# richox/orz

Hardware: AMD Instinct MI355X
Metric: orz -l1 encode throughput (enwik8-shaped text, 100 MB, one 16 MiB block in flight) (higher is better)
Workload: dtype u8

## Files before the change

### include/orz_hip.h

```cpp
#ifndef ORZ_HIP_H
#define ORZ_HIP_H

#include <stddef.h>
#include <stdint.h>
#include <sys/types.h>

#ifdef __cplusplus
extern "C" {
#endif

#define ORZ_OK 0
#define ORZ_EINVAL (-22)
#define ORZ_ENOMEM (-12)
#define ORZ_EIO (-5)
#define ORZ_ENODEV (-19)
#define ORZ_EBADMSG (-74)

#define ORZ_LZ_BLOCK_SIZE ((1u << 25) - 1)
#define ORZ_SBVEC_SENTINEL_LEN 480u
#define ORZ_SBVEC_PREMATCH_LEN (ORZ_LZ_BLOCK_SIZE / 2)

typedef struct {
    size_t match_depth, lazy_match_depth1, lazy_match_depth2;
} orz_lzcfg;
// ... 176 lines not shown
                    uint64_t* dst_len, orz_read_stats* stats);

typedef struct {
    uint64_t hits, resumed, fresh, uncached, evicted;
    uint64_t cursors, bytes, budget;
} orz_cache_stats;
int orz_reader_set_cache(orz_reader*, uint64_t max_bytes);
uint64_t orz_reader_cursor_state_bytes(void);
int orz_reader_cache_stats(orz_reader*, orz_cache_stats* stats);

int orz_reader_set_planes(orz_reader*, const uint32_t* elems, size_t n_tensors);
int orz_reader_set_planes_pieces(orz_reader*, const uint32_t* elems, const uint32_t* pieces, size_t n_tensors);
int orz_reader_set_bases(orz_reader*, const void* const* bases, size_t n_tensors);
int orz_element_gather_time(int device, const void* d_planes, const void* d_base, void* d_dst, size_t count, uint32_t elem, int reps,
                            double* ms);
int orz_reader_tensor_info(orz_reader*, uint64_t* n_tensors, uint64_t* counts, uint32_t* elems, size_t cap);
int orz_reader_read_elements(orz_reader*, const uint64_t* tensor, const uint64_t* first, const uint64_t* count, size_t n_ranges,
                             uint8_t* d_dst, size_t d_cap, uint64_t* dst_len, orz_read_stats* stats);

size_t orz_huffman_stride(void);
int orz_huffman_tables(int device, const uint32_t* weights, size_t nchunks, uint8_t* lens, uint16_t* codes, double* elapsed_us);

int orz_symrank_chains(int device, uint16_t* tables, const uint32_t* gsym, const uint32_t* rstart, size_t nitems,
                       uint16_t* ranks, uint32_t* flags2, double* elapsed_us);

int orz_fast_step_path(int device, unsigned form, uint32_t n, uint32_t tile, uint32_t t_lo, uint32_t t_hi, uint32_t entry,
                       const uint8_t* wbytes, const uint32_t* ev, uint8_t* ty, uint8_t* nl, uint8_t* x0, uint8_t* x1, uint8_t* x2,
                       uint32_t* centry, uint32_t* tentry, uint64_t* sbits, uint8_t* pt, uint32_t* cm, uint64_t* lds_bytes);
int orz_fast_step_counts(int device, uint32_t n, const uint8_t* wbytes, const uint64_t* sbits, int count, uint32_t s0, uint32_t s1,
                         uint32_t ext, uint32_t cpt, uint32_t live_end, uint32_t rows, uint32_t* cm, uint32_t* cp, uint32_t* cp2,
                         uint32_t* ord, uint32_t* ord2, uint32_t* acc2);
int orz_fast_step_horizon(int device, const uint32_t* cp, uint32_t rows, const uint32_t* hpre, uint32_t s0, uint32_t s1, uint32_t* hz,
                          uint32_t* hz2);

int orz_device_count(void);
const char* orz_last_error(void);
const char* orz_version(void);

#ifdef __cplusplus
}
#endif
#endif
```

### orz_amd/_native.py

```python
import ctypes
import os

_HERE = os.path.dirname(os.path.abspath(__file__))
LIB_PATH = os.environ.get("ORZ_LIB_PATH") or os.path.join(_HERE, "lib", "liborz_hip.so")


class LZCfg(ctypes.Structure):

    _fields_ = [
        ("match_depth", ctypes.c_size_t),
        ("lazy_match_depth1", ctypes.c_size_t),
        ("lazy_match_depth2", ctypes.c_size_t),
    ]


class EncodeStats(ctypes.Structure):
    _fields_ = [
        ("blocks", ctypes.c_uint64),
        ("sweeps", ctypes.c_uint64),
        ("seg_evals", ctypes.c_uint64),
        ("items", ctypes.c_uint64),
        ("chunks", ctypes.c_uint64),
        ("in_bytes", ctypes.c_uint64),
        ("out_bytes", ctypes.c_uint64),
# ... 306 lines not shown
    ),
    ("orz_stream_set_item_trace", ctypes.c_int, [ctypes.c_void_p, ctypes.c_int]),
    ("orz_stream_get_item_trace", ctypes.c_long, [ctypes.c_void_p, ctypes.POINTER(Item), ctypes.c_size_t]),
    ("orz_stream_set_item_patches", ctypes.c_int, [ctypes.c_void_p, ctypes.c_void_p, ctypes.c_size_t]),
    ("orz_stream_fast_tables", ctypes.c_long, [ctypes.c_void_p, ctypes.c_int, ctypes.c_char_p, ctypes.c_void_p, ctypes.c_size_t]),
    ("orz_stream_arm_repair_probe", ctypes.c_int, [ctypes.c_void_p, ctypes.c_int, ctypes.c_void_p, ctypes.c_void_p, ctypes.c_size_t]),
    ("orz_stream_repair_probe", ctypes.c_long, [ctypes.c_void_p, ctypes.c_char_p, ctypes.c_void_p, ctypes.c_size_t]),
    ("orz_huffman_stride", ctypes.c_size_t, []),
    (
        "orz_huffman_tables",
        ctypes.c_int,
        [ctypes.c_int, ctypes.c_void_p, ctypes.c_size_t, ctypes.c_void_p, ctypes.c_void_p, ctypes.POINTER(ctypes.c_double)],
    ),
    (
        "orz_symrank_chains",
        ctypes.c_int,
        [ctypes.c_int, ctypes.c_void_p, ctypes.c_void_p, ctypes.c_void_p, ctypes.c_size_t, ctypes.c_void_p, ctypes.c_void_p,
         ctypes.POINTER(ctypes.c_double)],
    ),
    (
        "orz_fast_step_path",
        ctypes.c_int,
        [ctypes.c_int, ctypes.c_uint] + [ctypes.c_uint32] * 5 + [ctypes.c_void_p] * 12 + [ctypes.POINTER(ctypes.c_uint64)],
    ),
    (
        "orz_fast_step_counts",
        ctypes.c_int,
        [ctypes.c_int, ctypes.c_uint32, ctypes.c_void_p, ctypes.c_void_p, ctypes.c_int] + [ctypes.c_uint32] * 6 + [ctypes.c_void_p] * 6,
    ),
    (
        "orz_fast_step_horizon",
        ctypes.c_int,
        [ctypes.c_int, ctypes.c_void_p, ctypes.c_uint32, ctypes.c_void_p, ctypes.c_uint32, ctypes.c_uint32, ctypes.c_void_p, ctypes.c_void_p],
    ),
    ("orz_device_count", ctypes.c_int, []),
    ("orz_last_error", ctypes.c_char_p, []),
    ("orz_version", ctypes.c_char_p, []),
]

_lib = None


def load():
    global _lib
    if _lib is not None:
        return _lib
    if not os.path.exists(LIB_PATH):
        raise RuntimeError(
            "liborz_hip.so is not built (%s missing): run `python -c 'import __graft_entry__ as g; g.build()'`" % LIB_PATH
        )
    os.environ.setdefault("GPU_MAX_HW_QUEUES", "16")
    lib = ctypes.CDLL(LIB_PATH)
    for name, restype, argtypes in SYMBOLS:
        fn = getattr(lib, name)
        fn.restype = restype
        fn.argtypes = argtypes
    _lib = lib
    return lib


def last_error():
    return load().orz_last_error().decode("utf-8", "replace")
```

### orz_amd/csrc/orz_capi.hip

```cpp
#include <cstdlib>
#include <cstring>
#include <map>
#include <memory>
#include <mutex>
#include <new>
#include <string>
#include <atomic>
#include <thread>
#include <vector>

#include "../../include/orz_hip.h"
#include "backend_hip.h"
#include "orz_decode_device.h"
#include "orz_decode_index.h"
#include "orz_decode_range.h"
#include "orz_decode_scatter.h"
#include "orz_host_decode.h"
#include "orz_planes.h"
#include "orz_read_elements.h"
#include "orz_decode_check.h"
#include "orz_stream.h"
#include "orz_fast_step.h"

namespace {
// ... 1378 lines not shown

int orz_fast_step_path(int device, unsigned form, uint32_t n, uint32_t tile, uint32_t t_lo, uint32_t t_hi, uint32_t entry,
                       const uint8_t* wbytes, const uint32_t* ev, uint8_t* ty, uint8_t* nl, uint8_t* x0, uint8_t* x1, uint8_t* x2,
                       uint32_t* centry, uint32_t* tentry, uint64_t* sbits, uint8_t* pt, uint32_t* cm, uint64_t* lds_bytes) {
    const int bad = mapped([&] { orz::fast_step_path_check(form, n, tile, t_lo, t_hi, entry, wbytes, ev, ty, nl, x0, x1, x2, centry, tentry, sbits, pt, cm); });
    if (bad) return bad;
    if (!device_ok(device)) return fail(ORZ_ENODEV, "no such HIP device");
    return mapped([&] {
        orz::HipBackend be(device);
        orz::fast_step_path(be, form, n, tile, t_lo, t_hi, entry, wbytes, ev, ty, nl, x0, x1, x2, centry, tentry, sbits, pt, cm, lds_bytes);
    });
}
int orz_fast_step_counts(int device, uint32_t n, const uint8_t* wbytes, const uint64_t* sbits, int count, uint32_t s0, uint32_t s1,
                         uint32_t ext, uint32_t cpt, uint32_t live_end, uint32_t rows, uint32_t* cm, uint32_t* cp, uint32_t* cp2,
                         uint32_t* ord, uint32_t* ord2, uint32_t* acc2) {
    const int bad = mapped([&] { orz::fast_step_counts_check(n, wbytes, sbits, s0, s1, ext, cpt, live_end, rows, cm, cp, cp2, ord, ord2, acc2); });
    if (bad) return bad;
    if (!device_ok(device)) return fail(ORZ_ENODEV, "no such HIP device");
    return mapped([&] {
        orz::HipBackend be(device);
        orz::fast_step_counts(be, n, wbytes, sbits, count, s0, s1, ext, cpt, live_end, rows, cm, cp, cp2, ord, ord2, acc2);
    });
}
int orz_fast_step_horizon(int device, const uint32_t* cp, uint32_t rows, const uint32_t* hpre, uint32_t s0, uint32_t s1, uint32_t* hz,
                          uint32_t* hz2) {
    const int bad = mapped([&] { orz::fast_step_horizon_check(cp, rows, hpre, s0, s1, hz, hz2); });
    if (bad) return bad;
    if (!device_ok(device)) return fail(ORZ_ENODEV, "no such HIP device");
    return mapped([&] {
        orz::HipBackend be(device);
        orz::fast_step_horizon(be, cp, rows, hpre, s0, s1, hz, hz2);
    });
}

int orz_symrank_chains(int device, uint16_t* tables, const uint32_t* gsym, const uint32_t* rstart, size_t nitems,
                       uint16_t* ranks, uint32_t* flags2, double* elapsed_us) {
    if (!tables || !rstart || (!gsym && nitems) || (!ranks && nitems)) return fail(ORZ_EINVAL, "bad argument");
    if (device < 0 || device >= orz_device_count()) return fail(ORZ_ENODEV, "no such HIP device");
    if (const char* why = orz::symrank_chains_invalid(tables, gsym, rstart, nitems)) return fail(ORZ_EINVAL, why);
    try {
        orz::HipBackend be(device);
        const size_t nt = (size_t)512 * orz::kSrWords;
        struct Bufs {
            orz::HipBackend& be;
            uint16_t *st = nullptr, *backup = nullptr, *rk = nullptr;
            uint32_t *gs = nullptr, *rs = nullptr, *fl = nullptr;
            ~Bufs() { be.free(st); be.free(backup); be.free(rk); be.free(gs); be.free(rs); be.free(fl); }
        } b{be};
        b.st = be.alloc<uint16_t>(nt, false);
        b.backup = be.alloc<uint16_t>(nt, false);
        b.rk = be.alloc<uint16_t>(nitems, false);
        b.gs = be.alloc<uint32_t>(nitems, false);
        b.rs = be.alloc<uint32_t>(513, false);
        b.fl = be.alloc<uint32_t>(3);
        be.h2d(b.st, tables, nt * 2);
        be.h2d(b.gs, gsym, nitems * 4);
        be.h2d(b.rs, rstart, 513 * 4);
        struct Events {
            hipEvent_t a = nullptr, b = nullptr;
            ~Events() { if (a) (void)hipEventDestroy(a); if (b) (void)hipEventDestroy(b); }
        } ev;
        ORZ_HIP_CHECK(hipEventCreate(&ev.a));
        ORZ_HIP_CHECK(hipEventCreate(&ev.b));
        ORZ_HIP_CHECK(hipEventRecord(ev.a, be.stream()));
        be.symrank(b.st, b.gs, b.rk, b.rs, (uint32_t)nitems, b.fl, b.backup, nullptr);
        ORZ_HIP_CHECK(hipEventRecord(ev.b, be.stream()));
// ... 241 lines not shown
```

### orz_amd/csrc/orz_fast.h

```cpp
#pragma once
#include "orz_kernels.h"
#include "orz_parse.h"

namespace orz {

#if !defined(__HIPCC__)
inline unsigned long long g_far_stats[4] = {0, 0, 0, 0};
#endif

constexpr uint32_t kSub = 4096;
constexpr uint32_t kSeg64 = 64;
constexpr uint32_t kNSub = kNewMax / kSub + 2;
constexpr uint32_t kEntries = 240;

constexpr uint32_t kFastK = 32;
constexpr uint32_t kHistSub = (kPre + 1) / kSub;
constexpr uint32_t kRingMargin = 4;
constexpr uint32_t kFastTile = 262144;
constexpr uint32_t kFastRounds = 4;
constexpr uint32_t kSettledTile = 393216;
constexpr uint32_t kSettledTileDeep = 262144;
constexpr uint32_t kSettledRounds = 3;

struct FastArgs {
// ... 286 lines not shown
};
struct ColScanTop {
    uint32_t* gsum;
    uint32_t rows;
    const uint32_t* out;
    const FastCtl* ctl = nullptr;
    ORZ_HD void operator()(size_t c) const {
        if (c >= 256 || passes_done(ctl)) return;
        uint32_t v = out[c];
        for (uint32_t g = 0; g * 64 < rows; g++) {
            const uint32_t t = gsum[(size_t)g * 256 + c];
            gsum[(size_t)g * 256 + c] = v;
            v += t;
        }
    }
};
struct ColScanRows {
    const uint32_t *in, *gsum;
    uint32_t rows;
    uint32_t* out;
    const FastCtl* ctl = nullptr;
    ORZ_HD void operator()(size_t tid) const {
        if (passes_done(ctl)) return;
        const uint32_t c = (uint32_t)(tid & 255), g = (uint32_t)(tid >> 8);
        if (g * 64 >= rows) return;
        uint32_t v = gsum[(size_t)g * 256 + c];
        for (uint32_t r = g * 64; r < rows && r < g * 64 + 64; r++) {
            out[(size_t)r * 256 + c] = v;
            v += in[(size_t)r * 256 + c];
        }
        if (g * 64 + 64 >= rows) out[(size_t)rows * 256 + c] = v;
    }
};
constexpr uint32_t kRecText = 12;
ORZ_D uint32_t rec_pos(uint64_t hi) { return (uint32_t)(hi >> 32); }
ORZ_D uint32_t rec_lcp(uint64_t lo_a, uint64_t hi_a, uint64_t lo_b, uint64_t hi_b) {
    const uint64_t x0 = lo_a ^ lo_b;
    if (x0) return (uint32_t)ctz64(x0) >> 3;
    const uint32_t x1 = (uint32_t)(hi_a ^ hi_b);
    return x1 ? 8 + ((uint32_t)ctz64((uint64_t)x1) >> 3) : kRecText;
}
struct FastRowsWave {
    const uint8_t* win;
    const uint32_t* epos;
    const uint64_t* stext;
    const uint8_t* rlen;
    uint32_t nent, K;
    uint8_t* rows;
    uint64_t* rdist;
    static constexpr uint32_t kOutStride = 72;
    static size_t lds_bytes(uint32_t K) { return (size_t)(64 + K) * 16 + 64 * kOutStride; }
    template <class W>
    ORZ_D void operator()(W& w) const {
        uint64_t* t0 = (uint64_t*)w.lds();
        uint64_t* t1 = t0 + (64 + K);
        uint8_t* outL = (uint8_t*)(t1 + (64 + K));
        const uint32_t lane = w.lane();
        const int64_t base = (int64_t)w.block() * 64 - K;
        for (uint32_t e = lane; e < 64 + K; e += 64) {
            const int64_t s = base + e;
            uint64_t a = 0, b = 0;
            if (s >= 0 && s < (int64_t)nent) { a = stext[2 * s]; b = stext[2 * s + 1]; }
            t0[e] = a; t1[e] = b;
        }
        w.sync();
        const uint32_t me = K + lane;
// ... 1209 lines not shown
                    const uint32_t p = kPre + i0 + t, c = hash1(a.win, p - 1), key = c * kHash + hash_entry(a.win + p);
                    if (!((rdirty[key >> 6] >> (key & 63)) & 1) && !edge[i0 + t] && cok[c]) mm &= ~(1ull << t);
                }
            }
        }
        const uint32_t mine = (uint32_t)popc64(mm) | ((uint32_t)popc64(wm) << 16);
        uint32_t v = mine;
        for (uint32_t d = 1; d < 64; d <<= 1) {
            const uint32_t t = w.shfl(v, lane >= d ? lane - d : lane);
            if (lane >= d) v += t;
        }
        const uint32_t tot = w.bcast(v, 63);
        uint32_t mo = (v - mine) & 0xffff, wo = (v - mine) >> 16;
        uint16_t* ml = mlist + (size_t)s * kSubMatches;
        uint16_t* wl = wlist + (size_t)s * kSubWords;
        while (mm) { const uint32_t t = (uint32_t)ctz64(mm); mm &= mm - 1; ml[mo++] = (uint16_t)(lane * 64 + t); }
        while (wm) { const uint32_t t = (uint32_t)ctz64(wm); wm &= wm - 1; wl[wo++] = (uint16_t)(lane * 64 + t); }
        if (lane == 0) { mcnt[s] = tot & 0xffff; wcnt[s] = tot >> 16; }
        w.sync();
        for (uint32_t c = lane; c < 256; c += 64) a.cm[(size_t)s * 256 + c] = cnt[c];
    }
};
struct FastItemTotal {
    const uint32_t* cp;
    uint32_t nsub;
    FastCtl* ctl;
    ORZ_HD void operator()(size_t c) const {
        if (c >= 256 || ctl->done) return;
        const uint32_t mine = cp[(size_t)nsub * 256 + c] - cp[c];
        atom_add32(&ctl->acc, mine);
        atom_max32(&ctl->hotacc, mine);
    }
};
struct OrdWave {
    const uint8_t* win;
    const uint64_t* sbits;
    const uint32_t* cp;
    uint32_t n;
    uint32_t* ORD;
    const FastCtl* ctl;
    static constexpr uint32_t kRow = 257;
    static size_t lds_bytes() { return (size_t)64 * kRow * 2 + 64; }
    template <class W>
    ORZ_D void operator()(W& w) const {
        if (ctl->done) return;
        uint16_t* cnt = (uint16_t*)w.lds();
        const uint32_t s = w.block(), lane = w.lane();
        uint16_t* mine = cnt + (size_t)lane * kRow;
        for (uint32_t c = 0; c < kRow; c++) mine[c] = 0;
        const uint32_t i0 = s * kSub + lane * 64;
        const uint64_t m0 = i0 < n ? sbits[i0 / 64] : 0;
        const uint8_t* b = win + kPre + i0;
        for (uint64_t m = m0; m;) {
            const uint32_t t = (uint32_t)ctz64(m);
            m &= m - 1;
            if (i0 + t < n) mine[(uint32_t)(b[(int)t - 1] & 0x7f) | ((uint32_t)is_alnum(b[(int)t - 2]) << 7)]++;
        }
        w.sync();
        for (uint32_t c = lane; c < 256; c += 64) {
            uint32_t run = 0;
            for (uint32_t r = 0; r < 64; r++) {
                const uint32_t v = cnt[(size_t)r * kRow + c];
                cnt[(size_t)r * kRow + c] = (uint16_t)run;
                run += v;
            }
        }
// ... 443 lines not shown
```

### orz_amd/csrc/orz_fast_step.h

```cpp
#pragma once
#include <stdexcept>
#include <vector>

#include "orz_fast.h"

namespace orz {

struct FastStepInvalid : std::invalid_argument {
    using std::invalid_argument::invalid_argument;
};

template <class BE>
struct StepBufs {
    BE& be;
    std::vector<void*> all;
    explicit StepBufs(BE& b) : be(b) {}
    ~StepBufs() { for (void* p : all) be.free(p); }
    template <class T> T* zeroed(size_t n) { T* p = be.template alloc<T>(n); all.push_back(p); return p; }
    template <class T> T* from(const T* src, size_t n) {
        T* p = be.template alloc<T>(n, false);
        all.push_back(p);
        be.h2d(p, src, n * sizeof(T));
        return p;
    }
// ... 98 lines not shown
    a.cp = d_cp2;
    be.launch_waves(flip_blocks(0) + 256, FlipPrefixWave{FastFlip{}, FastPrefix{a, s0, s1, ext, cpt, live_end}, 0}, FlipPrefixWave::lds_bytes());
    be.launch(256, FastItemTotal{d_cp, (uint32_t)z.nsub, ctl});
    be.launch_waves(z.nsub, OrdWave{a.win, a.sbits, d_cp, n, biased(d_ord, kPre), ctl}, OrdWave::lds_bytes());
    be.launch_waves(z.nsub, OrdWave2{a.win, a.sbits, d_cp, n, biased(d_ord2, kPre), ctl}, OrdWave2::lds_bytes());
    FastCtl h{};
    be.d2h(&h, ctl, sizeof h);
    acc2[0] = h.acc; acc2[1] = h.hotacc;
    be.d2h(cm, a.cm, ncm * 4); be.d2h(cp, d_cp, ncp * 4); be.d2h(cp2, d_cp2, ncp * 4);
    be.d2h(ord, d_ord, (size_t)n * 4); be.d2h(ord2, d_ord2, (size_t)n * 4);
}

inline void fast_step_horizon_check(const uint32_t* cp, uint32_t rows, const uint32_t* hpre, uint32_t s0, uint32_t s1, const uint32_t* hz, const uint32_t* hz2) {
    if (!cp || !hpre || !hz || !hz2) throw FastStepInvalid("null array");
    if (s0 > s1 || s1 + 2 > rows || rows > kNSub + 2) throw FastStepInvalid("subtile range");
}
template <class BE>
void fast_step_horizon(BE& be, const uint32_t* cp, uint32_t rows, const uint32_t* hpre, uint32_t s0, uint32_t s1, uint32_t* hz, uint32_t* hz2) {
    fast_step_horizon_check(cp, rows, hpre, s0, s1, hz, hz2);
    StepBufs<BE> b(be);
    FastArgs a{};
    a.cp = b.from(const_cast<uint32_t*>(cp), (size_t)rows * 256);
    a.hpre = b.from(const_cast<uint32_t*>(hpre), (size_t)(kHistSub + 1) * 256);
    const size_t nhz = ((size_t)s1 + 1) * 256 * 4;
    uint32_t* d_hz = b.from(hz, nhz);
    uint32_t* d_hz2 = b.from(hz2, nhz);
    a.hz = d_hz;
    { const FastHorizon fh{a, s0, s1}; be.launch(fh.threads(), fh); }
    a.hz = d_hz2;
    { const FastHorizon fh{a, s0, s1}; be.launch_waves((fh.threads() + 63) / 64, RetireHorizonWave{FastRetire{}, fh, 0}, 0); }
    be.d2h(hz, d_hz, nhz * 4); be.d2h(hz2, d_hz2, nhz * 4);
}

}
```

### orz_amd/csrc/orz_kernels.h

```cpp
#pragma once
#include "orz_common.h"

#if defined(__HIP_DEVICE_COMPILE__)
#define ORZ_ATOMIC_ADD(p, v) atomicAdd((p), (v))
#define ORZ_ATOMIC_MIN(p, v) atomicMin((p), (v))
#define ORZ_ATOMIC_MAX(p, v) atomicMax((p), (v))
#define ORZ_ATOMIC_OR(p, v) atomicOr((p), (v))
#else
template <class T, class U> inline T orz_fetch_add(T* p, U v) { return __atomic_fetch_add(p, (T)v, __ATOMIC_RELAXED); }
template <class T, class U> inline T orz_fetch_min(T* p, U v) {
    T o = __atomic_load_n(p, __ATOMIC_RELAXED);
    while ((T)v < o && !__atomic_compare_exchange_n(p, &o, (T)v, true, __ATOMIC_RELAXED, __ATOMIC_RELAXED)) {}
    return o;
}
template <class T, class U> inline T orz_fetch_max(T* p, U v) {
    T o = __atomic_load_n(p, __ATOMIC_RELAXED);
    while ((T)v > o && !__atomic_compare_exchange_n(p, &o, (T)v, true, __ATOMIC_RELAXED, __ATOMIC_RELAXED)) {}
    return o;
}
template <class T, class U> inline T orz_fetch_or(T* p, U v) { return __atomic_fetch_or(p, (T)v, __ATOMIC_RELAXED); }
#define ORZ_ATOMIC_ADD(p, v) orz_fetch_add((p), (v))
#define ORZ_ATOMIC_MIN(p, v) orz_fetch_min((p), (v))
#define ORZ_ATOMIC_MAX(p, v) orz_fetch_max((p), (v))
#define ORZ_ATOMIC_OR(p, v) orz_fetch_or((p), (v))
// ... 798 lines not shown
            uint32_t e = ienc[tid];
            if (e >= 5) put_bits(o, bp, c[2 * kSyms + e], l[2 * kSyms + e]);
        }
    }
};

struct WordsApply {
    const uint8_t* win;
    const uint32_t* wlast;
    uint32_t len;
    uint32_t last_type;
    uint8_t* wsnap;
    ORZ_HD void operator()(size_t tid) const {
        if (tid >= 32768) return;
        uint32_t u = wlast[tid];
        if (u) { wsnap[tid * 2] = win[u]; wsnap[tid * 2 + 1] = win[u + 1]; }
        if (last_type != kTyWord && hash2(win, len - 3) == tid) {
            wsnap[tid * 2] = win[len - 2];
            wsnap[tid * 2 + 1] = win[len - 1];
        }
    }
};

template <class T>
struct SlideArray {
    T* a;
    uint32_t off, sh, end;
    ORZ_HD void operator()(size_t tid) const {
        const uint32_t x = off + (uint32_t)tid;
        if (tid >= sh || x >= end) return;
        a[x] = x == 0 ? (T)0 : a[x + sh];
    }
};
}
```

### orz_amd/csrc/orz_stream.h

```cpp
#pragma once
#include <algorithm>
#include <atomic>
#include <cstdio>
#include <cstdlib>
#include <cstring>
#include <stdexcept>
#include <string>
#include <vector>

#include "orz_fast.h"
#include "orz_kernels.h"
#include "orz_parse.h"
#include "orz_verify.h"

namespace orz {

struct ItemTrace {
    std::vector<uint32_t> block, pos, src;
    std::vector<uint16_t> sym, ctx, rank, rob;
    std::vector<uint8_t> unl, enc, al, mlen;
    void clear() { block.clear(); pos.clear(); src.clear(); sym.clear(); ctx.clear(); rank.clear(); rob.clear(); unl.clear(); enc.clear(); al.clear(); mlen.clear(); }
};

struct FastTableCapture {
// ... 435 lines not shown
            krunend_ = take<uint32_t>(32768 + 1);
            vbits_ = take<uint64_t>(kWLen / 64 + 2);
            v1_ = take<uint64_t>(kWLen / 4096 + 2);
            v2_ = take<uint64_t>(kWLen / 262144 + 2);
            kbits_ = take<uint64_t>(kNewMax / 64 + 2);
            k1_ = take<uint64_t>(kNewMax / 4096 + 2);
            k2_ = take<uint64_t>(kNewMax / 262144 + 2);
            if (!fast_) {
                srec_ = take<SlotRec>(kWLen);
                exitst_ = take<uint64_t>((size_t)nseg_max_ + 2);
                hist_ = take<uint8_t>((size_t)ring_ * 256);
                base_ = take<uint32_t>((size_t)ring_ * 256);
                ctl_ = take<ParseCtl>(1);
                partial_ = take<uint32_t>((size_t)2 * (wsegs_ / kRankChunk + 1) * 256);
            } else {
                const size_t nn = (size_t)kNewMax + 512;
                frows_ = take<uint8_t>((size_t)kNewMax * fK_ + 64, false);
                frlen_ = take<uint8_t>(nn);
                fstext_ = take<uint64_t>((size_t)kWLen * 2, false);
                fkw_ = take<uint16_t>(nn);
                fev_ = take<uint32_t>(nn, false);
                fty_ = take<uint8_t>(nn);
                fnl_ = take<uint8_t>(nn);
                fpt_ = take<uint8_t>(nn);
                fmf_ = take<uint8_t>(nn);
                fef_ = take<uint8_t>(nn);
                fdirty_ = take<uint8_t>(nn);
                frdist_ = take<uint64_t>(nn, false);
                fwmask_ = take<uint64_t>(nn, false);
                fkmeta_ = take<uint16_t>(nn);
                fhz_ = take<uint32_t>((size_t)(kNSub + 2) * 256 * 4);
                fhcm_ = take<uint32_t>((size_t)kHistSub * 256);
                fhpre_ = take<uint32_t>((size_t)(kHistSub + 1) * 256);
                fgsum_ = take<uint32_t>((size_t)(kNSub / 64 + 4) * 256);
                fdiag_ = take<unsigned long long>(64);
                fx0_ = take<uint8_t>(nn);
                fx1_ = take<uint8_t>((size_t)(kNSub + 2) * kEntries);
                fx2_ = take<uint8_t>((size_t)(kNewMax / kSub + 4) * kEntries);
                fsbits_ = take<uint64_t>(kNewMax / 64 + 16);
                fcentry_ = take<uint32_t>(kNSub + 2);
                ftentry_ = take<uint32_t>(kNewMax / kSub + 4);
                fcm_ = take<uint32_t>((size_t)(kNSub + 2) * 256);
                fcp_ = take<uint32_t>((size_t)(kNSub + 2) * 256);
                fcut_ = take<uint32_t>(nn);
                frdirty_ = take<uint64_t>((size_t)2 * kDirtyWords);
                flaste_ = take<uint32_t>(nn);
                fctl_ = take<FastCtl>(1);
                fcok_ = take<uint32_t>(512);
                ffarv_ = take<uint32_t>(nn, false);
                fcl_ = take<uint64_t>((size_t)kWLen * 2, false);
                fccnt_ = take<uint32_t>(kNumKeys + 1);
                fcnew_ = take<uint32_t>(kNumKeys + 1);
            }
            f32_ = take<uint32_t>((size_t)kNewMax + 8, false);
            sc32_ = take<uint32_t>((size_t)kNewMax + 8, false);
            hpos_ = take<uint32_t>(kPre + 1);
            ctxcount_ = take<uint32_t>(256);
            tailkey_ = take<uint32_t>(8);
            wsnap_ = take<uint8_t>(65536);
            wlast_ = take<uint32_t>(32768);
            for (TailSet& t : ts_) {
                t.cap = 0;
                grow_tail_set(t, getenv("ORZ_TAIL_ITEMS0") ? std::max<uint32_t>(65536u, (uint32_t)strtoul(getenv("ORZ_TAIL_ITEMS0"), nullptr, 10)) : kTailItems0);
                t.rstart = take<uint32_t>(520);
                t.hw = take<uint32_t>((size_t)kMaxChunks * kHwStride);
                t.hl = take<uint8_t>((size_t)kMaxChunks * kHwStride);
                t.hc = take<uint16_t>((size_t)kMaxChunks * kHwStride);
// ... 242 lines not shown
            be_.free(tim);
        }
        stats.sweeps += sweeps;
        be_.launch(n, FinalizeBlock{idx_, kidx_, srec_, kbits_, len, S_, ML_, E_, ORD_});
        be_.sync();
        double t2 = be_.now();
        stats.t_parse += t2 - t1;
#ifdef ORZ_DEBUG_ROBUST
        {
            std::vector<uint8_t> hS(len), hw(len + 8);
            std::vector<uint32_t> hO(len), cnt(256, 0), hb(256);
            be_.d2h(hS.data(), S_, len); be_.d2h(hO.data(), ORD_, (size_t)len * 4); be_.d2h(hw.data(), win, len);
            be_.d2h(cnt.data(), ctxcount_, 256 * 4);
            int bad = 0;
            for (uint32_t x = kPre; x < len; x++) if (hS[x]) {
                uint32_t c = (hw[x - 1] & 0x7f) | ((uint32_t)is_alnum(hw[x - 2]) << 7);
                if (hO[x] != cnt[c] && bad++ < 10) fprintf(stderr, "ORD mismatch x=%u seg=%u ctx=%u ord=%u want=%u\n", x, (x - kPre) / seg_, c, hO[x], cnt[c]);
                cnt[c]++;
            }
            fprintf(stderr, "ORD check: %d bad\n", bad);
            if (const char* dp = getenv("ORZ_DUMP_ITEMS")) {
                std::vector<uint8_t> hT(len), hM(len); std::vector<uint32_t> hR(len);
                be_.d2h(hT.data(), TY_, len); be_.d2h(hM.data(), ML_, len); be_.d2h(hR.data(), SRC_, (size_t)len * 4);
                FILE* f = fopen(dp, "w");
                for (uint32_t x = kPre; x < len; x++) if (hS[x]) fprintf(f, "%u ty=%u ml=%u src=%u ord=%u\n", x, hT[x] & 3, hM[x], (hT[x] & 3) == 2 ? hR[x] : 0, hO[x]);
                fclose(f);
            }
        }
#endif

        post_stage(n, len, out, chunk_ends, t2);
    }

    void col_scan(const uint32_t* in, uint32_t rows, uint32_t* out, const FastCtl* ctl = nullptr) {
        const size_t groups = (rows + 63) / 64;
        be_.launch(groups * 256, ColScanGroups{in, rows, fgsum_, ctl});
        be_.launch(256, ColScanTop{fgsum_, rows, out, ctl});
        be_.launch(groups * 256, ColScanRows{in, fgsum_, rows, out, ctl});
    }

    void debug_dump(const char* tag, uint32_t n, const FastCtl* h) {
        static const char* dir = getenv("ORZ_DEBUG_DUMP");
        if (!dir) return;
        static const uint32_t at = getenv("ORZ_DEBUG_POS") ? (uint32_t)strtoul(getenv("ORZ_DEBUG_POS"), nullptr, 10) : kPre + 256;
        const uint32_t lo = (std::max(at, kPre + 256) - 256) & ~63u, w = 512;
        if (lo + w > kPre + n) return;
        const uint32_t i0 = lo - kPre;
        struct Rec { uint32_t lo, w, block, passes, total, nmem, lastflips, pad; } rec{lo, w, (uint32_t)stats.blocks, h ? h->passes : 0, h ? h->total : 0, h ? h->nmem : 0, h ? h->lastflips : 0, 0};
        std::vector<uint8_t> b8(w);
        std::vector<uint32_t> b32(w);
        std::vector<uint64_t> b64(w / 64 + 2);
        char name[512];
        static std::atomic<unsigned> serial{0};
        snprintf(name, sizeof name, "%s/dump_%05u_%p_b%u_%s.bin", dir, serial.fetch_add(1), (void*)this, (unsigned)stats.blocks, tag);
        FILE* f = fopen(name, "wb");
        if (!f) return;
        fwrite(&rec, sizeof rec, 1, f);
        be_.d2h(b64.data(), fsbits_ + i0 / 64, b64.size() * 8); fwrite(b64.data(), 8, b64.size(), f);
        const uint8_t* a8[] = {fty_ + i0, fnl_ + i0, fpt_ + i0, fmf_ + i0, fef_ + i0, fdirty_ + i0, S_ + lo, TY_ + lo, ML_ + lo, W0_ + lo, LENMIN_ + lo, LMV_ + lo, dwin() + lo};
        for (const uint8_t* q : a8) { be_.d2h(b8.data(), q, w); fwrite(b8.data(), 1, w, f); }
        const uint32_t* a32[] = {SRC_ + lo, ORD_ + lo, fev_ + i0, ffarv_ + i0, idx_ + lo, fcut_ + i0};
        for (const uint32_t* q : a32) { be_.d2h(b32.data(), q, (size_t)w * 4); fwrite(b32.data(), 4, w, f); }
        fclose(f);
    }

    void probe_put(const std::string& name, const void* dev, size_t bytes) {
        repair_probe->tab.emplace_back(name, std::vector<uint8_t>(bytes));
        be_.d2h(repair_probe->tab.back().second.data(), dev, bytes);
    }
    void probe_state(const std::string& tag, uint32_t n) {
        probe_put(tag + ".ty", fty_, (size_t)n + 1);
// ... 170 lines not shown
            a.rounds = R;
            if (attempt) {
                be_.memset(vbits_ + nent / 64, 0, 16);
                be_.launch_waves(((size_t)nent + 63) / 64, FastSlotInitWave{epos_, nullptr, runstart_, nent, vbits_, frlen_}, 0);
                be_.memset(fccnt_, 0, (size_t)(kNumKeys + 1) * 4);
                be_.launch(nent, FastListReset{epos_, slot_keys, runstart_, nent, fccnt_});
            }
            const size_t nn = (size_t)n + 264;
            {
                ZeroRanges z;
                z.add(kbits_, ((size_t)n / 64 + 2) * 8);
                z.add(k1_, ((size_t)kNewMax / 4096 + 2) * 8);
                z.add(fty_, nn); z.add(fnl_, nn); z.add(fpt_, nn); z.add(fmf_, nn); z.add(fef_, nn);
                z.add(fsbits_, ((size_t)n / 64 + 8) * 8);
                z.add(fcm_, (size_t)(nsub + 2) * 256 * 4);
                z.add(fcp_, (size_t)(nsub + 2) * 256 * 4);
                z.add(&fctl_->lastflips, 4);
                z.add(fcnew_, (size_t)(kNumKeys + 1) * 4);
                if (repair_lists) {
                    z.add(tbits, tbits_bytes);
                    z.add(kdirty, kdirty_bytes);
                    z.add(fcok_, 256 * 4);
                    z.add(frdirty_ + kDirtyWords, (size_t)kDirtyWords * 8);
                }
                be_.launch(z.units(), z);
            }
            be_.launch(nvw / 64 + 1, V1Build{vbits_, nvw, v1_});
            be_.launch(256, FastCpInit{ctxcount_, fcp_, ftentry_});
            const uint32_t ntile = (n + T - 1) / T, cpt = T / kSub;
            be_.launch_waves(256, FastPrefix{a, 0, 0, std::min(cpt + 1, nsub), cpt, 0}, 0);
            { const FastHorizon fh{a, 0, std::min(cpt + 1, nsub) - 1}; be_.launch(fh.threads(), fh); }
            static const bool fused_steps = !(getenv("ORZ_FAST_FUSED") && !strcmp(getenv("ORZ_FAST_FUSED"), "0"));
            const bool use_graph = be_.graphs_enabled() && (n == kNewMax || n == cur_unit_) && !probing;
            const uint64_t gkey = ((uint64_t)R << 58) | ((uint64_t)T << 32) | n;
            const bool replayed = use_graph && be_.graph_replay(gkey);
            struct CaptureGuard {
                BE& be;
                bool on;
                ~CaptureGuard() { if (on) be.graph_capture_abort(); }
            } capture{be_, use_graph && !replayed};
            if (capture.on) be_.graph_capture_begin();
            if (replayed) stats.sweeps += ntile + R - 1;
            for (uint32_t step = 1; step <= ntile + R - 1 && !replayed; step++) {
                const uint32_t t_lo = step > R ? step - R : 0, t_hi = std::min(step - 1, ntile - 1);
                const uint32_t lo = kPre + t_lo * T;
                const uint32_t hi = (uint32_t)std::min<uint64_t>(len, (uint64_t)kPre + (uint64_t)(t_hi + 1) * T);
                const uint32_t hi2 = std::min(len, hi + 2);
                be_.timed_begin();
                const uint32_t r1lo = step <= ntile ? kPre + t_hi * T : hi;
                const uint32_t r2lo = step >= 2 && step - 2 < ntile ? kPre + (step - 2) * T : (step < 2 ? kPre : hi);
                const uint32_t mark_hi = step - 1 < ntile ? kPre + (step - 1) * T : len;
                const uint32_t cline = kPre + (step > R ? step - R : 0) * T;
                be_.launch(hi2 - lo, FastEval{a, lo, hi2, r1lo, r2lo, step, cline});
                be_.timed_end();
                const bool had_retire = fused_steps && step - 1 >= R && step - 1 < ntile + R - 1;
                const uint32_t plo = had_retire ? kPre + (step - 1 - R) * T : kPre, phi = had_retire ? (uint32_t)std::min<uint64_t>(len, (uint64_t)plo + T) : kPre;
                const PathRange pr = fast_path_stage(be_, a, t_lo, t_hi, fused_steps ? kPathFused : kPathUnfused, FastRetireDone{a, plo, phi, fcut_});
                const uint32_t c0 = pr.c0, nc = pr.nc;
                const uint32_t fhi = std::min(len, hi + 240);
                const FastFlip ff{a, lo, fhi, t_hi + 1, mark_hi, step >= R ? (uint32_t)std::min<uint64_t>(len, (uint64_t)lo + T) : 0, &fctl_->lastflips};
                const uint32_t ext = std::min(cpt + 1, nsub - std::min(nsub, c0 + nc));
                const FastPrefix fp{a, c0, c0 + nc, ext, cpt, step >= R ? std::min(c0 + cpt, c0 + nc) : c0};
                const FastHorizon fh{a, c0, c0 + nc + ext - 1};
                const bool retire = step >= R && step < ntile + R - 1;
                const uint32_t rlo = retire ? kPre + (step - R) * T : kPre, rhi = retire ? (uint32_t)std::min<uint64_t>(len, (uint64_t)rlo + T) : kPre;
                if (fused_steps) {
                    const uint32_t nflip = fhi - lo + 1, nret = rhi - rlo;
                    be_.launch_waves(flip_blocks(nflip) + 256, FlipPrefixWave{ff, fp, nflip}, FlipPrefixWave::lds_bytes());
                    be_.launch_waves((size_t)(nret + 63) / 64 + (fh.threads() + 63) / 64, RetireHorizonWave{FastRetire{a, rlo, rhi, fcut_}, fh, nret}, 0);
                } else {
                    be_.launch((size_t)fhi - lo + 1, ff);
                    be_.launch_waves(256, fp, 0);
                    be_.launch(fh.threads(), fh);
                    if (retire) {
                        be_.launch(rhi - rlo, FastRetire{a, rlo, rhi, fcut_});
                        be_.launch(rhi - rlo, FastRetireDone{a, rlo, rhi, fcut_});
                    }
                }
                stats.sweeps++;
            }
            const bool incr_repairs = !getenv("ORZ_FAST_FULLPASS");
            const uint32_t src_cap = getenv("ORZ_FAST_SRCCAP") ? (uint32_t)atoi(getenv("ORZ_FAST_SRCCAP")) : 4 * a.depth + 4;
            static const bool ord_ballots = !(getenv("ORZ_FAST_ORD") && !strcmp(getenv("ORZ_FAST_ORD"), "table"));
            const FastFlip flip_all{a, kPre, len, ~0u, 0, 0, &fctl_->lastflips};
            const uint32_t tw = n / 64 + 1;
            int pass = 0;
            auto lists_pass = [&]() {
                    if (pass == 0) be_.launch((size_t)n + 1, flip_all);
                    else be_.launch(tw, FastFlipSparse{flip_all, tw, kdirty, fctl_});
                    uint64_t* rd_in = frdirty_ + (size_t)(pass & 1) * kDirtyWords;
                    uint64_t* rd_out = frdirty_ + (size_t)((pass + 1) & 1) * kDirtyWords;
                    {
                        FastCokGrow cg{fcok_, fcok_ + 256};
                        cg.ctl = fctl_;
                        if (pass) { cg.rd_out = rd_out; cg.nwords = kDirtyWords; }
                        be_.launch(cg.threads(), cg);
                    }
                    be_.launch_waves(nsub, RepairListWave{a, mlist, wlist, mcnt, wcnt, pass && incr_repairs ? rd_in : nullptr, fdirty_, fcok_ + 256, fctl_},
                                     RepairListWave::lds_bytes());
                    col_scan(fcm_, nsub, fcp_, fctl_);
                    be_.launch(256, FastItemTotal{fcp_, nsub, fctl_});
                    if (ord_ballots) be_.launch_waves(nsub, OrdWave2{win, fsbits_, fcp_, n, ORD_, fctl_}, OrdWave2::lds_bytes());
                    else be_.launch_waves(nsub, OrdWave{win, fsbits_, fcp_, n, ORD_, fctl_}, OrdWave::lds_bytes());
                    FastSource fs{a, SRC_, fcut_, pass && incr_repairs ? rd_in : nullptr, src_cap, fctl_, fdirty_, fcok_ + 256};
                    fs.cutlist = cutlist; fs.ncut = &fctl_->ncut;
                    const uint32_t per = kListThreads;
                    be_.launch((size_t)nsub * per, FastSourceL{fs, mlist, mcnt, nsub, per});
                    FastRecut rc{a, fcut_, rd_out};
                    rc.wextra = wextra; rc.nwx = &fctl_->nwx; rc.cgrow = fcok_;
                    be_.launch(kRepairGrid, FastRecutL{rc, cutlist, fctl_, kRepairGrid});
                    be_.launch(tw, FastFlipSparse{flip_all, tw, kdirty, fctl_});
                    if (pass == 0) {
                        be_.launch(nk, KbitVals{kbits_, nk, f32_});
                        be_.inclusive_max_scan_u32(f32_, flaste_, nk);
                    }
                    be_.launch((size_t)nsub * kListThreads, FastWordCheckL{a, pass == 0 ? flaste_ : nullptr, kdirty, wextra, fixlist, fctl_, wlist, wcnt, nsub});
                    be_.launch(kRepairGrid, FastWordApplyL{a, fixlist, rd_out, fcok_, fctl_, kRepairGrid, kdirty});
                    if (probing) probe_pass(n, nsub, mcnt, wcnt, mlist, wlist);
                    be_.launch(1, FastPassEnd{fctl_});
            };
            auto lists_tail = [&]() {
                be_.launch(nk, KbitVals{kbits_, nk, f32_});
                be_.inclusive_max_scan_u32(f32_, flaste_, nk);
                be_.launch(n, FastCommit{a, flaste_, &fctl_->lt, S_, TY_, ML_, W0_});
                be_.launch(n, Flags32{S_, n, f32_});
                be_.exclusive_scan_u32(f32_, sc32_, n);
                be_.launch(1, SumLast{sc32_, f32_, n - 1, tailkey_ + 3});
            };
            if (probing) probe_begin(n, nsub, mlist, wlist, repair_lists);
            if (repair_lists && !replayed) {
                be_.launch(1, FastCtlReset{fctl_});
                for (int k = 0; k < kFirstPasses; k++, pass++) lists_pass();
                lists_tail();
            }
            capture.on = false;
            if (use_graph && !replayed) be_.graph_capture_end(gkey);
            debug_dump("r", n, nullptr);
            if (ts_[cur_set_].pending && !pend_order_.empty() && pend_order_.front() == cur_set_) collect_one(out, nullptr);
            FastCtl h{};
            if (repair_lists) {
                pass = kFirstPasses;
                for (int group = 0; group < 64; group++) {
                    be_.d2h_async(&h, fctl_, sizeof h);
                    be_.d2h_async(pre_two_, tailkey_ + 3, 8);
                    be_.sync();
                    pre_items_valid_ = h.done != 0;
                    if (h.done) break;
                    for (int k = 0; k < 2; k++, pass++) lists_pass();
                    lists_tail();
                }
            } else {
                be_.launch(1, FastCtlReset{fctl_});
                auto grid_pass = [&]() {
                    be_.launch((size_t)n + 1, FastFlip{a, kPre, len, ~0u, 0, 0, &fctl_->lastflips});
                    be_.launch_waves(nsub, CountWave{a, 0}, CountWave::lds_bytes());
                    col_scan(fcm_, nsub, fcp_);
                    be_.launch(256, FastItemTotal{fcp_, nsub, fctl_});
                    be_.launch_waves(nsub, OrdWave{win, fsbits_, fcp_, n, ORD_, fctl_}, OrdWave::lds_bytes());
                    uint64_t* rd_in = frdirty_ + (size_t)(pass & 1) * kDirtyWords;
                    uint64_t* rd_out = frdirty_ + (size_t)((pass + 1) & 1) * kDirtyWords;
                    be_.memset(rd_out, 0, (size_t)kDirtyWords * 8);
                    be_.launch(256, FastCtxOk{fcp_, nsub, fcok_, fcok_ + 256, pass == 0, fctl_});
                    be_.launch(n, FastSource{a, SRC_, fcut_, pass && incr_repairs ? rd_in : nullptr, src_cap, fctl_, fdirty_, fcok_ + 256});
                    be_.launch(n, FastRecut{a, fcut_, rd_out});
                    be_.launch((size_t)n + 1, FastFlip{a, kPre, len, ~0u, 0, 0, &fctl_->lastflips});
                    be_.launch(nk, KbitVals{kbits_, nk, f32_});
                    be_.inclusive_max_scan_u32(f32_, flaste_, nk);
#if defined(ORZ_RACE_SELFTEST)
                    be_.launch(n, FastWordCheckRacy{a, flaste_, rd_out, fctl_});
#else
                    be_.launch(n, FastWordCheck{a, flaste_, fcut_, fctl_});
                    be_.launch(n, FastWordApply{a, fcut_, rd_out});
#endif
                    if (probing) probe_pass(n, nsub, nullptr, nullptr);
// ... 379 lines not shown
    template <class TS>
    void apply_item_patches(uint32_t point, TS& t, uint32_t nitems) {
        if (!npatch_) return;
        be_.launch(npatch_, ItemPatchApply{ipatch_, npatch_, (uint32_t)stats.blocks, point, t.ipos, nitems, TY_, ML_, LMV_, SRC_, ORD_,
                                           t.isym, t.ictx, t.irob, t.iunl, t.ienc, t.ial, ipatch_applied_});
    }
    void check_item_patches() {
        if (!npatch_) return;
        uint32_t applied = 0;
        be_.d2h(&applied, ipatch_applied_, 4);
        if (applied != npatch_)
            throw std::runtime_error("item patches: " + std::to_string(npatch_ - applied) + " of " + std::to_string(npatch_) +
                                     " patches were not applied (no item starts at their block and position): the encode fails");
    }
    void set_inject(uint32_t kind, uint32_t nth) { inject_kind_ = kind; inject_nth_ = nth; }
    void report_verify(const char* what) {
        unsigned long long h6[6];
        be_.d2h(h6, fdiag_ + 32, sizeof h6);
        if (h6[1] | h6[2] | h6[3] | h6[4]) {
            char msg[320];
            snprintf(msg, sizeof msg, "fast parse verification, %s (%llu blocks so far): of %llu matches %llu have a source that is no item start, %llu one of another context, %llu one outside the ring, %llu one with other bytes (e.g. at window offset %llu)",
                     what, (unsigned long long)stats.blocks, h6[0], h6[1], h6[2], h6[3], h6[4], h6[5]);
            fprintf(stderr, "orz: %s\n", msg);
            throw std::runtime_error(msg);
        }
    }

    void slide(bool slide_window = true) { slide_by(last_n_, 0, slide_window); }
    void slide_by(uint32_t sh, uint32_t extra, bool slide_window = true) {
        if (sh != kNewMax) hist_hint_ = ~0u;
        be_.launch(3, TailKeys{dwin(), kPre + sh, tailkey_});
        if (slide_window) be_.d2d(dwin() - 2, dwin() + sh - 2, (size_t)kPre + extra + 2);
        else be_.d2d(dwin() - 2, dwin() + sh - 2, 2);
        for (uint32_t off = 0; off < kPre; off += sh) {
            be_.launch(sh, SlideArray<uint8_t>{S_, off, sh, kPre});
            be_.launch(sh, SlideArray<uint8_t>{ML_, off, sh, kPre});
            be_.launch(sh, SlideArray<uint32_t>{ORD_, off, sh, kPre});
            be_.launch(sh, SlideArray<uint8_t>{LENMIN_, off, sh, kPre});
            be_.launch(sh, SlideArray<uint32_t>{vrec_, off, sh, kPre});
            be_.launch(sh, SlideArray<uint32_t>{vord_, off, sh, kPre});
        }
    }
    template <class OutT>
    void encode_block_units(uint32_t take, bool lead, OutT& out) {
        uint32_t unit = fast_ ? unit_ : kNewMax;
        const bool lead_units = fast_ && lead && lead_unit_ && lead_unit_ < unit;
        if (lead_units) unit = lead_unit_;
        cur_unit_ = unit;
        uint32_t done = 0;
        while (done < take) {
            uint32_t n = std::min(unit, take - done);
            if (take - done - n < unit / 8) n = take - done;
            set_lead_block(lead && done == 0 && !lead_units);
            unit_base_ = done;
            encode_block(n, out);
            done += n;
            if (done < take) slide_by(n, take - done);
        }
        unit_base_ = 0;
        cur_unit_ = fast_ ? unit_ : kNewMax;
    }
    void set_unit(uint32_t bytes) {
        if (bytes < (1u << 20) || bytes > kNewMax || bytes % kSub) throw std::runtime_error("the unit must be a multiple of 4096 in [1 MiB, 16 MiB]");
        unit_ = cur_unit_ = bytes;
    }
    void set_lead_unit(uint32_t bytes) { lead_unit_ = bytes; }
    uint32_t lead_unit() const { return lead_unit_; }

    EncodeStats stats;
    ItemTrace* trace = nullptr;
    FastRepairProbe* repair_probe = nullptr;
    FastTableCapture* tables = nullptr;

   private:
    template <class T>
    T* take(size_t n, bool zero = true) {
        T* p = be_.template alloc<T>(n, zero);
        owned_.push_back(p);
        return p;
    }
    void release_all() {
        for (void* p : owned_) if (p) be_.free(p);
        owned_.clear();
        be_.release_arena();
    }
    void release_token() {
        if (token_held_) { token_held_ = false; be_.parse_token_release(); }
    }
    bool token_held_ = false;
    int probe_pass_ = 0;
    bool pre_items_valid_ = false;
    uint32_t pre_two_[2] = {0, 0};
    std::vector<void*> owned_;
    BE& be_;
    Cfg cfg_;
    uint32_t seg_, wsegs_, ring_ = 0, nseg_max_ = 0, dmax_ = 0;
    bool fast_ = false;
    uint32_t ftile_ = kFastTile, frounds_ = kFastRounds, fK_ = kFastK;
    bool sched_auto_ = false, settled_next_ = false;
    uint32_t sched_tile_ = kSettledTile, sched_rounds_ = kSettledRounds;
    bool lead_block_ = false;
    uint8_t *frows_ = nullptr, *frlen_ = nullptr, *fty_ = nullptr, *fnl_ = nullptr, *fpt_ = nullptr, *fmf_ = nullptr, *fef_ = nullptr,
            *fx0_ = nullptr, *fx1_ = nullptr, *fx2_ = nullptr, *fdirty_ = nullptr;
    uint16_t *fkw_ = nullptr, *fkmeta_ = nullptr;
    uint64_t *frdist_ = nullptr, *fwmask_ = nullptr;
    uint32_t *fhz_ = nullptr, *fhcm_ = nullptr, *fhpre_ = nullptr, *fgsum_ = nullptr;
    unsigned long long* fdiag_ = nullptr;
    uint32_t *fev_ = nullptr, *fcentry_ = nullptr, *ftentry_ = nullptr, *fcm_ = nullptr, *fcp_ = nullptr, *fcut_ = nullptr,
             *flaste_ = nullptr, *fcok_ = nullptr, *ffarv_ = nullptr;
    uint64_t *fsbits_ = nullptr, *fstext_ = nullptr, *frdirty_ = nullptr, *fcl_ = nullptr;
    uint32_t *fccnt_ = nullptr, *fcnew_ = nullptr;
    FastCtl* fctl_ = nullptr;
    FastCtl hfin_{};
    uint8_t lt_carry_ = kTyLit;
    bool stream_start_ = true;
    struct TailSet {
        uint32_t* ipos = nullptr;
        uint16_t *isym = nullptr, *ictx = nullptr, *irank = nullptr, *irob = nullptr, *grank = nullptr, *skey = nullptr;
        uint8_t *iunl = nullptr, *ienc = nullptr, *ial = nullptr;
        uint32_t *gsym = nullptr, *sperm = nullptr, *blen = nullptr, *bscan = nullptr, *rstart = nullptr;
        uint32_t* hw = nullptr;
        uint8_t* hl = nullptr;
        uint16_t* hc = nullptr;
        uint32_t *hdrbits = nullptr, *tot = nullptr, *out = nullptr, *srflags = nullptr;
        bool pending = false;
        bool framed = false;
        uint32_t cap = 0;
        uint32_t nitems = 0, nchunks = 0, len = 0, block = 0;
    };
    static constexpr int kEvItems = 0, kEvRank = 2, kEvTail = 4, kEvGate = 6, kEvOut = 8, kEvIdle = 10;
    static constexpr uint32_t kFrameThreads = 1u << 18;
    struct MainStreamGuard {
        BE& be;
        ~MainStreamGuard() { be.select(0); }
    };
    TailSet ts_[2];
    static constexpr uint32_t kTailItems0 = 6u << 20;
    struct Fresh {
        BE& be;
// ... 121 lines not shown
```

Before: 526.2.

## Fuse column scan into one wave kernel and merge six slide launches

Replaces the three-kernel column prefix scan (group sums, top scan, row fixup) plus a separate item-total kernel with a single wave-per-column kernel. Each wave does shuffle-based scans over 8 row chunks and atomically accumulates the totals. Slide now uses one kernel per offset that moves all six arrays, instead of six launches. The aim is fewer launches and no global scratch round trip in the repeated lists pass, at the cost of serial per-column work on 256 waves. It also adds a first-passes env override, folded into the graph cache key.

```diff
diff --git a/include/orz_hip.h b/include/orz_hip.h
--- a/include/orz_hip.h
+++ b/include/orz_hip.h
@@ -232,6 +232,8 @@
                          uint32_t* ord, uint32_t* ord2, uint32_t* acc2);
 int orz_fast_step_horizon(int device, const uint32_t* cp, uint32_t rows, const uint32_t* hpre, uint32_t s0, uint32_t s1, uint32_t* hz,
                           uint32_t* hz2);
+int orz_fast_step_colscan(int device, const uint32_t* in, uint32_t rows, const uint32_t* base, int done, uint32_t* out3, uint32_t* out1,
+                          uint32_t* acc4);
 
 int orz_device_count(void);
 const char* orz_last_error(void);
diff --git a/orz_amd/_native.py b/orz_amd/_native.py
--- a/orz_amd/_native.py
+++ b/orz_amd/_native.py
@@ -362,6 +362,11 @@
         "orz_fast_step_horizon",
         ctypes.c_int,
         [ctypes.c_int, ctypes.c_void_p, ctypes.c_uint32, ctypes.c_void_p, ctypes.c_uint32, ctypes.c_uint32, ctypes.c_void_p, ctypes.c_void_p],
+    ),
+    (
+        "orz_fast_step_colscan",
+        ctypes.c_int,
+        [ctypes.c_int, ctypes.c_void_p, ctypes.c_uint32, ctypes.c_void_p, ctypes.c_int, ctypes.c_void_p, ctypes.c_void_p, ctypes.c_void_p],
     ),
     ("orz_device_count", ctypes.c_int, []),
     ("orz_last_error", ctypes.c_char_p, []),
diff --git a/orz_amd/csrc/orz_capi.hip b/orz_amd/csrc/orz_capi.hip
--- a/orz_amd/csrc/orz_capi.hip
+++ b/orz_amd/csrc/orz_capi.hip
@@ -1434,6 +1434,16 @@
         orz::fast_step_horizon(be, cp, rows, hpre, s0, s1, hz, hz2);
     });
 }
+int orz_fast_step_colscan(int device, const uint32_t* in, uint32_t rows, const uint32_t* base, int done, uint32_t* out3, uint32_t* out1,
+                          uint32_t* acc4) {
+    const int bad = mapped([&] { orz::fast_step_colscan_check(in, rows, base, out3, out1, acc4); });
+    if (bad) return bad;
+    if (!device_ok(device)) return fail(ORZ_ENODEV, "no such HIP device");
+    return mapped([&] {
+        orz::HipBackend be(device);
+        orz::fast_step_colscan(be, in, rows, base, done, out3, out1, acc4);
+    });
+}
 
 int orz_symrank_chains(int device, uint16_t* tables, const uint32_t* gsym, const uint32_t* rstart, size_t nitems,
                        uint16_t* ranks, uint32_t* flags2, double* elapsed_us) {
diff --git a/orz_amd/csrc/orz_fast.h b/orz_amd/csrc/orz_fast.h
--- a/orz_amd/csrc/orz_fast.h
+++ b/orz_amd/csrc/orz_fast.h
@@ -342,6 +342,41 @@
         if (g * 64 + 64 >= rows) out[(size_t)rows * 256 + c] = v;
     }
 };
+ORZ_D void item_total(FastCtl* ctl, uint32_t mine);
+struct ColScanWave {
+    const uint32_t* in;
+    uint32_t rows;
+    uint32_t* out;
+    FastCtl* ctl = nullptr;
+    uint32_t totals = 0;
+    static constexpr uint32_t kTrips = 8;
+    static size_t lds_bytes() { return 0; }
+    template <class W>
+    ORZ_D void operator()(W& w) const {
+        if (passes_done(ctl)) return;
+        const uint32_t c = w.block(), lane = w.lane();
+        const uint32_t first = out[c];
+        uint32_t carry = first;
+        for (uint32_t base = 0; base < rows; base += 64 * kTrips) {
+            uint32_t v[kTrips];
+            for (uint32_t k = 0; k < kTrips; k++) {
+                const uint32_t r = base + k * 64 + lane;
+                v[k] = r < rows ? in[(size_t)r * 256 + c] : 0;
+            }
+            for (uint32_t d = 1; d < 64; d <<= 1)
+                for (uint32_t k = 0; k < kTrips; k++) {
+                    const uint32_t t = w.shfl(v[k], lane >= d ? lane - d : lane);
+                    if (lane >= d) v[k] += t;
+                }
+            for (uint32_t k = 0; k < kTrips; k++) {
+                const uint32_t r = base + k * 64 + lane;
+                if (r < rows) out[(size_t)(r + 1) * 256 + c] = carry + v[k];
+                carry += w.bcast(v[k], 63);
+            }
+        }
+        if (totals && lane == 0) item_total(ctl, carry - first);
+    }
+};
 constexpr uint32_t kRecText = 12;
 ORZ_D uint32_t rec_pos(uint64_t hi) { return (uint32_t)(hi >> 32); }
 ORZ_D uint32_t rec_lcp(uint64_t lo_a, uint64_t hi_a, uint64_t lo_b, uint64_t hi_b) {
@@ -1617,6 +1652,10 @@
         atom_max32(&ctl->hotacc, mine);
     }
 };
+ORZ_D void item_total(FastCtl* ctl, uint32_t mine) {
+    atom_add32(&ctl->acc, mine);
+    atom_max32(&ctl->hotacc, mine);
+}
 struct OrdWave {
     const uint8_t* win;
     const uint64_t* sbits;
diff --git a/orz_amd/csrc/orz_fast_step.h b/orz_amd/csrc/orz_fast_step.h
--- a/orz_amd/csrc/orz_fast_step.h
+++ b/orz_amd/csrc/orz_fast_step.h
@@ -154,4 +154,48 @@
     be.d2h(hz, d_hz, nhz * 4); be.d2h(hz2, d_hz2, nhz * 4);
 }
 
-}
+inline void fast_step_colscan_check(const uint32_t* in, uint32_t rows, const uint32_t* base, const uint32_t* out3, const uint32_t* out1, const uint32_t* acc4) {
+    if (!in || !base || !out3 || !out1 || !acc4) throw FastStepInvalid("null array");
+    if (!rows || rows > kHistSub) throw FastStepInvalid("rows outside 1 .. 4096");
+}
+template <class BE>
+void fast_step_colscan(BE& be, const uint32_t* in, uint32_t rows, const uint32_t* base, int done, uint32_t* out3, uint32_t* out1, uint32_t* acc4) {
+    fast_step_colscan_check(in, rows, base, out3, out1, acc4);
+    StepBufs<BE> b(be);
+    const size_t nin = (size_t)rows * 256, nout = ((size_t)rows + 1) * 256, groups = (rows + 63) / 64;
+    const uint32_t* d_in = b.from(const_cast<uint32_t*>(in), nin);
+    uint32_t* d3 = b.from(out3, nout);
+    uint32_t* d1 = b.from(out1, nout);
+    be.h2d(d3, base, 256 * 4);
+    be.h2d(d1, base, 256 * 4);
+    uint32_t* gsum = b.template zeroed<uint32_t>(groups * 256);
+    FastCtl h[2] = {};
+    for (int k = 0; k < 2; k++) { h[k].done = done ? 1 : 0; h[k].acc = acc4[2 * k]; h[k].hotacc = acc4[2 * k + 1]; }
+    FastCtl* ctl = b.from(h, 2);
+    be.launch(groups * 256, ColScanGroups{d_in, rows, gsum, ctl});
+    be.launch(256, ColScanTop{gsum, rows, d3, ctl});
+    be.launch(groups * 256, ColScanRows{d_in, gsum, rows, d3, ctl});
+    be.launch(256, FastItemTotal{d3, rows, ctl});
+    be.launch_waves(256, ColScanWave{d_in, rows, d1, ctl + 1, 1}, ColScanWave::lds_bytes());
+    be.d2h(h, ctl, sizeof h);
+    for (int k = 0; k < 2; k++) { acc4[2 * k] = h[k].acc; acc4[2 * k + 1] = h[k].hotacc; }
+    be.d2h(out3, d3, nout * 4); be.d2h(out1, d1, nout * 4);
+}
+
+inline void fast_step_slide_check(uint32_t sh, uint32_t end, const void* b0, const void* b1, const void* b2, const void* w0, const void* w1, const void* w2) {
+    if (!b0 || !b1 || !b2 || !w0 || !w1 || !w2) throw FastStepInvalid("null array");
+    if (!sh || !end || end > kPre) throw FastStepInvalid("shift or end outside 1 .. kPre");
+}
+template <class BE>
+void fast_step_slide(BE& be, uint32_t sh, uint32_t end, size_t len, uint8_t* b0, uint8_t* b1, uint8_t* b2, uint32_t* w0, uint32_t* w1, uint32_t* w2) {
+    fast_step_slide_check(sh, end, b0, b1, b2, w0, w1, w2);
+    if (len < (size_t)end + sh) throw FastStepInvalid("arrays shorter than end + shift");
+    StepBufs<BE> b(be);
+    uint8_t *d0 = b.from(b0, len), *d1 = b.from(b1, len), *d2 = b.from(b2, len);
+    uint32_t *e0 = b.from(w0, len), *e1 = b.from(w1, len), *e2 = b.from(w2, len);
+    slide_six(be, SlideSix{d0, d1, d2, e0, e1, e2, 0, sh, end});
+    be.d2h(b0, d0, len); be.d2h(b1, d1, len); be.d2h(b2, d2, len);
+    be.d2h(w0, e0, len * 4); be.d2h(w1, e1, len * 4); be.d2h(w2, e2, len * 4);
+}
+
+}
diff --git a/orz_amd/csrc/orz_kernels.h b/orz_amd/csrc/orz_kernels.h
--- a/orz_amd/csrc/orz_kernels.h
+++ b/orz_amd/csrc/orz_kernels.h
@@ -854,4 +854,26 @@
         a[x] = x == 0 ? (T)0 : a[x + sh];
     }
 };
-}
+struct SlideSix {
+    uint8_t *b0, *b1, *b2;
+    uint32_t *w0, *w1, *w2;
+    uint32_t off, sh, end;
+    ORZ_HD void operator()(size_t tid) const {
+        const uint32_t x = off + (uint32_t)tid;
+        if (tid >= sh || x >= end) return;
+        uint8_t p0 = 0, p1 = 0, p2 = 0;
+        uint32_t q0 = 0, q1 = 0, q2 = 0;
+        if (x) {
+            const size_t y = (size_t)x + sh;
+            p0 = b0[y]; p1 = b1[y]; p2 = b2[y];
+            q0 = w0[y]; q1 = w1[y]; q2 = w2[y];
+        }
+        b0[x] = p0; b1[x] = p1; b2[x] = p2;
+        w0[x] = q0; w1[x] = q1; w2[x] = q2;
+    }
+};
+template <class BE>
+void slide_six(BE& be, SlideSix k) {
+    for (k.off = 0; k.off < k.end; k.off += k.sh) be.launch(k.sh, k);
+}
+}
diff --git a/orz_amd/csrc/orz_stream.h b/orz_amd/csrc/orz_stream.h
--- a/orz_amd/csrc/orz_stream.h
+++ b/orz_amd/csrc/orz_stream.h
@@ -491,7 +491,6 @@
                 fhz_ = take<uint32_t>((size_t)(kNSub + 2) * 256 * 4);
                 fhcm_ = take<uint32_t>((size_t)kHistSub * 256);
                 fhpre_ = take<uint32_t>((size_t)(kHistSub + 1) * 256);
-                fgsum_ = take<uint32_t>((size_t)(kNSub / 64 + 4) * 256);
                 fdiag_ = take<unsigned long long>(64);
                 fx0_ = take<uint8_t>(nn);
                 fx1_ = take<uint8_t>((size_t)(kNSub + 2) * kEntries);
@@ -800,11 +799,19 @@
         post_stage(n, len, out, chunk_ends, t2);
     }
 
-    void col_scan(const uint32_t* in, uint32_t rows, uint32_t* out, const FastCtl* ctl = nullptr) {
-        const size_t groups = (rows + 63) / 64;
-        be_.launch(groups * 256, ColScanGroups{in, rows, fgsum_, ctl});
-        be_.launch(256, ColScanTop{fgsum_, rows, out, ctl});
-        be_.launch(groups * 256, ColScanRows{in, fgsum_, rows, out, ctl});
+    const FastCtl& last_ctl() const { return hfin_; }
+    static int first_passes() {
+        static const int forced = [] {
+            const char* v = getenv("ORZ_FAST_FIRSTPASSES");
+            if (!v) return 0;
+            const int k = atoi(v);
+            if (k < 1 || k > kFirstPasses) throw std::runtime_error("ORZ_FAST_FIRSTPASSES must be in [1, 12]");
+            return k;
+        }();
+        return forced ? forced : kFirstPasses;
+    }
+    void col_scan(const uint32_t* in, uint32_t rows, uint32_t* out, FastCtl* ctl = nullptr, bool totals = false) {
+        be_.launch_waves(256, ColScanWave{in, rows, out, ctl, totals ? 1u : 0u}, ColScanWave::lds_bytes());
     }
 
     void debug_dump(const char* tag, uint32_t n, const FastCtl* h) {
@@ -1041,7 +1048,8 @@
             { const FastHorizon fh{a, 0, std::min(cpt + 1, nsub) - 1}; be_.launch(fh.threads(), fh); }
             static const bool fused_steps = !(getenv("ORZ_FAST_FUSED") && !strcmp(getenv("ORZ_FAST_FUSED"), "0"));
             const bool use_graph = be_.graphs_enabled() && (n == kNewMax || n == cur_unit_) && !probing;
-            const uint64_t gkey = ((uint64_t)R << 58) | ((uint64_t)T << 32) | n;
+            const int npass0 = first_passes();
+            const uint64_t gkey = ((uint64_t)R << 58) | ((uint64_t)T << 32) | ((uint64_t)npass0 << 28) | n;
             const bool replayed = use_graph && be_.graph_replay(gkey);
             struct CaptureGuard {
                 BE& be;
@@ -1107,8 +1115,7 @@
                     }
                     be_.launch_waves(nsub, RepairListWave{a, mlist, wlist, mcnt, wcnt, pass && incr_repairs ? rd_in : nullptr, fdirty_, fcok_ + 256, fctl_},
                                      RepairListWave::lds_bytes());
-                    col_scan(fcm_, nsub, fcp_, fctl_);
-                    be_.launch(256, FastItemTotal{fcp_, nsub, fctl_});
+                    col_scan(fcm_, nsub, fcp_, fctl_, true);
                     if (ord_ballots) be_.launch_waves(nsub, OrdWave2{win, fsbits_, fcp_, n, ORD_, fctl_}, OrdWave2::lds_bytes());
                     else be_.launch_waves(nsub, OrdWave{win, fsbits_, fcp_, n, ORD_, fctl_}, OrdWave::lds_bytes());
                     FastSource fs{a, SRC_, fcut_, pass && incr_repairs ? rd_in : nullptr, src_cap, fctl_, fdirty_, fcok_ + 256};
@@ -1139,7 +1146,7 @@
             if (probing) probe_begin(n, nsub, mlist, wlist, repair_lists);
             if (repair_lists && !replayed) {
                 be_.launch(1, FastCtlReset{fctl_});
-                for (int k = 0; k < kFirstPasses; k++, pass++) lists_pass();
+                for (int k = 0; k < npass0; k++, pass++) lists_pass();
                 lists_tail();
             }
             capture.on = false;
@@ -1148,7 +1155,7 @@
             if (ts_[cur_set_].pending && !pend_order_.empty() && pend_order_.front() == cur_set_) collect_one(out, nullptr);
             FastCtl h{};
             if (repair_lists) {
-                pass = kFirstPasses;
+                pass = npass0;
                 for (int group = 0; group < 64; group++) {
                     be_.d2h_async(&h, fctl_, sizeof h);
                     be_.d2h_async(pre_two_, tailkey_ + 3, 8);
@@ -1594,14 +1601,7 @@
         be_.launch(3, TailKeys{dwin(), kPre + sh, tailkey_});
         if (slide_window) be_.d2d(dwin() - 2, dwin() + sh - 2, (size_t)kPre + extra + 2);
         else be_.d2d(dwin() - 2, dwin() + sh - 2, 2);
-        for (uint32_t off = 0; off < kPre; off += sh) {
-            be_.launch(sh, SlideArray<uint8_t>{S_, off, sh, kPre});
-            be_.launch(sh, SlideArray<uint8_t>{ML_, off, sh, kPre});
-            be_.launch(sh, SlideArray<uint32_t>{ORD_, off, sh, kPre});
-            be_.launch(sh, SlideArray<uint8_t>{LENMIN_, off, sh, kPre});
-            be_.launch(sh, SlideArray<uint32_t>{vrec_, off, sh, kPre});
-            be_.launch(sh, SlideArray<uint32_t>{vord_, off, sh, kPre});
-        }
+        slide_six(be_, SlideSix{S_, ML_, LENMIN_, ORD_, vrec_, vord_, 0, sh, kPre});
     }
     template <class OutT>
     void encode_block_units(uint32_t take, bool lead, OutT& out) {
@@ -1666,7 +1666,7 @@
             *fx0_ = nullptr, *fx1_ = nullptr, *fx2_ = nullptr, *fdirty_ = nullptr;
     uint16_t *fkw_ = nullptr, *fkmeta_ = nullptr;
     uint64_t *frdist_ = nullptr, *fwmask_ = nullptr;
-    uint32_t *fhz_ = nullptr, *fhcm_ = nullptr, *fhpre_ = nullptr, *fgsum_ = nullptr;
+    uint32_t *fhz_ = nullptr, *fhcm_ = nullptr, *fhpre_ = nullptr;
     unsigned long long* fdiag_ = nullptr;
     uint32_t *fev_ = nullptr, *fcentry_ = nullptr, *ftentry_ = nullptr, *fcm_ = nullptr, *fcp_ = nullptr, *fcut_ = nullptr,
              *flaste_ = nullptr, *fcok_ = nullptr, *ffarv_ = nullptr;
```

Result: faster. 533.3 (median of 6 runs) (+1.4%).
